# adalkiran/llama-nuts-and-bolts

Measured on AMD Instinct MI355X. Metric: decode tokens/s Llama-3.1-8B bf16 @1/2/4/8 MI355X; % HBM roofline, higher is better.
Workload: dtype bf16; 1 GPU; Llama-3.1-8B bf16, 1xMI355X, single-prompt greedy decode, seq_len=128 -> +125 tokens (configs[1]'s prompt, --steps 125); prompt_len=128, sequences_in_flight=1, parallelism=single GPU, mode=exact-order (token-id identical to the CPU reference path), reported_repeat=median, weight_bytes_resident=16060522496

## Files before the change

llama-nuts-and-bolts_amd/csrc/lnb_api.cpp:

```cpp
#include <hip/hip_runtime.h>
#include <algorithm>
#include <array>
#include <cmath>
#include <cstdarg>
#include <cstdio>
#include <cstdlib>
#include <cstring>
#include <chrono>
#include <dirent.h>
#include <unistd.h>
#include <deque>
#include <map>
#include <mutex>
#include <string>
#include <vector>
#include "../../include/lnb.h"
#include "lnb_device.h"
#include "lnb_knobs.h"
#include "lnb_kvcopy.h"
#include "lnb_rowpack.h"
#include "lnb_batchplan.h"
#include "lnb_rccl.h"
static_assert(LNB_MAX_SEQ_LEN == LNB_SEQ_MAX, "lnb.h and lnb_device.h disagree on the longest context");
static_assert(ROWPACK_MAX_W == LNB_BATCH_MAX, "lnb_rowpack.h and lnb_device.h disagree on the columns of a pass");
static_assert(BATCHPLAN_COLS == LNB_STREAM_COLS, "lnb_batchplan.h and lnb_device.h disagree on the sequences of a column group");
static_assert(LNB_MAX_FORK == KVC_MAX_DST, "lnb.h and lnb_kvcopy.h disagree on the destinations of a fork");
static_assert(LNB_MAX_TOP_K == LNB_TOKPROB_MAX_K, "lnb.h and lnb_device.h disagree on the largest top-k");
static_assert(LNB_MAX_DRAFT == LNB_SPEC_MAX_DRAFT && LNB_MAX_DRAFT + 1 <= LNB_STREAM_COLS, "a verify pass is one column group of at most 16 columns");

extern "C" {
hipError_t lnbk_gemv(const GemvParams* p, int rw, int nch, int epi, int norm, hipStream_t st);
hipError_t lnbk_attn(const AttnParams* p, hipStream_t st);
hipError_t lnbk_attn_rows(const AttnParams* p, int pos0, hipStream_t st);
int lnbk_attn_short_max_T(int hd);
size_t lnbk_attn_long_lds(int seq_len);
size_t lnbk_attn_long_layout_lds(int seq_len);
size_t lnbk_attn_one_lds(int seq_len, int hd);
hipError_t lnbk_exp_table(double* tab, float divisor, hipStream_t st);
hipError_t lnbk_gemm(const GemmParams* p, int epi, hipStream_t st);
hipError_t lnbk_rmsnorm_rows(const uint16_t* x, const uint16_t* w, uint16_t* out, int S, int K, float eps, hipStream_t st);
hipError_t lnbk_embed(const uint16_t* emb, const int32_t* tokens, uint16_t* x, int S, int dim, int vocab, int* err, hipStream_t st);
hipError_t lnbk_argmax(const uint16_t* logits, int V, int32_t* next_token, StepState* state, int32_t* out_tokens, int out_cap, int advance, hipStream_t st);
hipError_t lnbk_set_state(StepState* state, int pos, int n_out, int honour_stop, hipStream_t st);
hipError_t lnbk_set_stop(StepState* state, const int32_t* ids, int n, hipStream_t st);
hipError_t lnbk_advance_state(StepState* state, int rows, hipStream_t st);
hipError_t lnbk_tile(const uint16_t* src, uint16_t* dst, int rows, int K, int row_off, int chain, int RW, int NCH, int gather, hipStream_t st);
// ... 885 lines not shown

enum { K_QKV = 0, K_ATTN = 1, K_WO = 2, K_W13 = 3, K_W2 = 4, K_HEAD = 5, K_LAYER = 6 };
static bool use_mfma(int S) { return knob(Knob::PREFILL_MFMA) && S >= 16; }
static GemmParams gemm_of(const TiledDesc& t, const uint16_t* x, int K, int n_rows, int S, const StepState* st) {
    GemmParams g{}; g.w = t.w; g.rw = t.rw; g.nch = t.nch; g.x = x; g.K = K; g.n_rows = n_rows; g.S = S; g.st = st; g.w16 = t.w16; return g;
}
static hipError_t gemv_dispatch(const lnb_ctx* c, const GemvParams* g, int rw, int nch, int epi, int norm, hipStream_t st) {
    return c->mode == LNB_MODE_FAST ? lnbk_fast_gemv(g, rw, nch, epi, norm, st) : lnbk_gemv(g, rw, nch, epi, norm, st);
}
static hipError_t gemm_dispatch(int mode, const GemmParams* g, int epi, hipStream_t st) {
    if (mode == LNB_MODE_FAST && g->S >= knob(Knob::FAST_GEMM_MIN_ROWS)) { hipError_t e = lnbk_fast_gemm(g, epi, st); if (e != hipErrorNotSupported) return e; }
    if (knob(Knob::PREFILL_STREAM) && (g->K & 127) == 0 && (g->w16 || (knob(Knob::PREFILL_NATIVE) && g->w && (g->rw == 4 ? g->nch == 1 && (epi == EPI_STORE || epi == EPI_RESID) : g->rw >= 16))))
        return lnbk_gemm_stream(g, epi, g_num_cus, st);
    return lnbk_gemm(g, epi, st);
}
static int enqueue_layer_kernel(lnb_ctx* c, int l, int S, int which, hipStream_t st_other = nullptr, int lds_pad = 0) {
    lnb_model* m = c->m; const lnb_model_args& a = m->a; hipStream_t st = st_other ? st_other : c->stream;
    LayerW& L = m->layers[l - m->layer_begin];
    uint16_t* ck = c->ck[l - m->layer_begin]; uint16_t* cv = c->cv[l - m->layer_begin];
    uint16_t* const hbuf = m->whole(l) ? c->h : c->x;
    if (use_mfma(S) && which != K_ATTN) {
        switch (which) {
        case K_QKV: {
            HIPCHK(lnbk_rmsnorm_rows(c->x, L.attn_norm, c->xn, S, a.dim, a.norm_eps, st));
            GemmParams g = gemm_of(L.wqkv, c->xn, a.dim, L.wqkv.n_rows, S, c->st);
            g.cis = m->cis; g.q_out = c->q; g.cache_k = ck; g.cache_v = cv; g.seq_len = c->seq_len; g.q_dim = m->q_dim; g.kv_dim = m->kv_dim; g.head_dim = m->head_dim;
            HIPCHK(gemm_dispatch(c->mode, &g, EPI_QKV_ROPE, st)); return 0; }
        case K_WO: { GemmParams g = gemm_of(L.wo, c->att, m->q_dim, a.dim, S, c->st); g.out = hbuf; g.res = c->x; HIPCHK(gemm_dispatch(c->mode, &g, EPI_RESID, st)); return 0; }
        case K_W13: {
            HIPCHK(lnbk_rmsnorm_rows(hbuf, L.ffn_norm, c->xn, S, a.dim, a.norm_eps, st));
// ... 4 lines not shown
    }
    switch (which) {
    case K_QKV: {
        GemvParams g{}; g.w = L.wqkv.w; g.x = c->x; g.norm_w = L.attn_norm; g.norm_fb = c->zseq_count + 1; g.eps = a.norm_eps; g.K = a.dim; g.n_rows = L.wqkv.n_rows; g.S = S; g.st = c->st;
        g.cis = m->cis; g.q_out = c->q; g.cache_k = ck; g.cache_v = cv; g.seq_len = c->seq_len; g.q_dim = m->q_dim; g.kv_dim = m->kv_dim; g.head_dim = m->head_dim;
        g.sched = c->sched;
        set_grid(g, L.wqkv); HIPCHK(gemv_dispatch(c, &g, L.wqkv.rw, 1, EPI_QKV_ROPE, 1, st)); return 0; }
    case K_ATTN: {
        AttnParams ap{}; ap.q = c->q; ap.cache_k = ck; ap.cache_v = cv; ap.out = c->att; ap.st = c->st; ap.dbg = g_dbg;
        ap.S = S; ap.H = a.n_heads; ap.KVH = a.n_kv_heads; ap.hd = m->head_dim; ap.seq_len = c->seq_len;
        ap.lds_T = c->seq_len < c->attn_short_cap ? c->seq_len : c->attn_short_cap;
        ap.host_T = c->call_T;
        ap.divisor = bf_wide_h(bf_trunc_h((float)std::sqrt((double)m->head_dim)));
        ap.mfma = use_mfma(S) ? 1 : 0; ap.exp_tab = m->exp_tab;
        ap.causal = (c->attn_causal && S > 1) ? 1 : 0;
        ap.longctx = 0; ap.force_zseq = c->force_zseq & 1; ap.e_buf = c->e_buf; ap.z_part = c->z_part; ap.zseq_count = c->zseq_count; ap.cnt = c->attn_cnt;
        if (ap.mfma && c->sidx_jt > 0 && c->call_T > 0 && c->sidx_jt * 16 >= c->call_T) { ap.score_idx = c->score_idx; ap.sidx_jt = c->sidx_jt; }
        if (S == 1 && c->attn_long) {
            const bool one = (knob(Knob::ATTN_ONE) || (c->force_zseq & 12)) && !(c->force_zseq & 2) && c->sched == LNB_SCHED_LATENCY && m->head_dim % 16 == 0 &&
                             a.n_heads * (m->head_dim / 16) <= g_num_cus && lnbk_attn_one_lds(c->seq_len, m->head_dim) <= (size_t)160 * 1024;
            ap.longctx = one ? ((c->force_zseq & 4) ? 3 : 2) : 1;
        }
        if (c->attn_rows && ap.causal) {
            ap.e_buf = c->sp_e_buf; ap.z_part = c->sp_z_part; ap.force_zseq = c->rows_flags & 1;
            HIPCHK(lnbk_attn_rows(&ap, c->call_T - S, st)); return 0;
        }
        if (c->mode == LNB_MODE_FAST && ap.mfma) {
            hipError_t e = lnbk_fast_attn(&ap, st);
            if (e != hipErrorNotSupported) { HIPCHK(e); return 0; }
        }
        HIPCHK(lnbk_attn(&ap, st)); return 0; }
    case K_WO: {
        GemvParams o{}; o.w = L.wo.w; o.x = c->att; o.K = m->q_dim; o.n_rows = a.dim; o.S = S; o.st = c->st; o.out = hbuf; o.res = c->x; o.sched = c->sched;
        set_grid(o, L.wo); HIPCHK(gemv_dispatch(c, &o, L.wo.rw, 1, EPI_RESID, 0, st)); return 0; }
    case K_W13: {
        GemvParams f{}; f.w = L.w13.w; f.x = hbuf; f.norm_w = L.ffn_norm; f.norm_fb = c->zseq_count + 1; f.eps = a.norm_eps; f.K = a.dim; f.n_rows = m->ffn_hidden; f.S = S; f.st = c->st;
        f.out = c->ffn; f.silu = m->silu; f.sched = c->sched;
        set_grid(f, L.w13); HIPCHK(gemv_dispatch(c, &f, L.w13.rw, 2, EPI_SILU_MUL, 1, st)); return 0; }
    case K_W2: {
        GemvParams d{}; d.w = L.w2.w; d.x = c->ffn; d.K = m->ffn_hidden; d.n_rows = a.dim; d.S = S; d.st = c->st; d.out = c->x; d.res = hbuf; d.lds_pad = lds_pad; d.sched = c->sched; d.prio = knob(Knob::W2_PRIO);
        set_grid(d, L.w2); HIPCHK(gemv_dispatch(c, &d, L.w2.rw, 1, EPI_RESID, 0, st)); return 0; }
    }
    return fail("bad kernel id");
}
static int enqueue_layers(lnb_ctx* c, int S, bool with_cb) {
    lnb_model* m = c->m;
    for (int l = m->layer_begin; l < m->layer_end; l++) {
        auto t0 = std::chrono::steady_clock::now();
        for (int k = K_QKV; k <= K_W2; k++) {
            if (!(k <= K_WO ? m->has_attn(l) : k == K_W13 ? m->has_w13(l) : m->has_w2(l))) continue;
            if (enqueue_layer_kernel(c, l, S, k)) return -1;
        }
        if (with_cb && c->cb) {
            HIPCHK(hipStreamSynchronize(c->stream));
            double secs = std::chrono::duration<double>(std::chrono::steady_clock::now() - t0).count();
// ... 2129 lines not shown
```

llama-nuts-and-bolts_amd/csrc/lnb_device.h:

```cpp
#pragma once
#include <stdint.h>
#include <stddef.h>

#if defined(__HIPCC__)
#define LNB_HD __host__ __device__ __forceinline__
#else
#define LNB_HD inline
#endif

struct TiledDesc {
    uint16_t* w;
    int n_rows;
    int k;
    int rw;
    int nch;
    int n_blocks;
    uint16_t* w16;
};
LNB_HD size_t tiled_index(int n, int k, int c, int K, int RW, int NCH) {
    if (RW == 4) return ((((size_t)(n >> 2) * (size_t)(K >> 7) + (size_t)(k >> 7)) * 64 + (size_t)((n & 3) * 16 + (k & 15))) << 3) + (size_t)((k & 127) >> 4);
    size_t b = (size_t)(n / RW), r = (size_t)(n % RW), kc = (size_t)(k >> 3), e = (size_t)(k & 7);
    return ((((b * (size_t)(K >> 3) + kc) * (size_t)NCH + (size_t)c) * (size_t)RW + r) << 3) + e;
}
LNB_HD size_t tiled_elems(int n_rows, int K, int RW, int NCH) {
    if (RW == 4) return (size_t)((n_rows + 15) / 16) * 16 * (size_t)K;
    return (size_t)((n_rows + RW - 1) / RW) * (size_t)RW * (size_t)NCH * (size_t)K;
}

LNB_HD uint64_t lnb_splitmix64(uint64_t z) {
    z += 0x9E3779B97F4A7C15ULL;
    z = (z ^ (z >> 30)) * 0xBF58476D1CE4E5B9ULL;
    z = (z ^ (z >> 27)) * 0x94D049BB133111EBULL;
    return z ^ (z >> 31);
}
LNB_HD int32_t lnb_synth_isum(uint64_t base, uint64_t idx) {
    uint64_t a = lnb_splitmix64(base ^ idx);
    uint64_t b = lnb_splitmix64(a);
    int32_t s = 0;
    for (int i = 0; i < 4; i++) { s += (int32_t)((a >> (16 * i)) & 0xFFFF); s += (int32_t)((b >> (16 * i)) & 0xFFFF); }
    return s - 262140;
}

// ... 23 lines not shown
    uint16_t* out;
    const uint16_t* res;
    const float* silu;
    const float* cis;
    uint16_t* q_out;
    uint16_t* cache_k;
    uint16_t* cache_v;
    int seq_len;
    int q_dim, kv_dim, head_dim;
    long long* dbg;
    int dbg_full;
    int* norm_fb;
    int lds_pad;
    int prio;
    int sched;
};

struct GemmParams {
    const uint16_t* w;
    int rw, nch;
    const uint16_t* x;
    int K, n_rows, S;
    const StepState* st;
    uint16_t* out; const uint16_t* res; const float* silu;
    const float* cis; uint16_t* q_out; uint16_t* cache_k; uint16_t* cache_v; int seq_len, q_dim, kv_dim, head_dim;
    const uint16_t* w16;
    const struct BatchTab* btab; const struct BatchKV* bkv;
    uint16_t* out_xt;
    int rows_fastest;
};
// ... 12 lines not shown
    int mfma;
    const double* exp_tab;
    int longctx;
    int force_zseq;
    double* e_buf;
    double* z_part;
    int pw_floats;
    int* zseq_count;
    unsigned* cnt;
    const struct BatchTab* btab; const struct BatchKV* bkv; uint16_t* out_xt;
    uint64_t* score_idx;
    int sidx_jt;
    int touch;
    int causal;
    int head_major;
};
constexpr int LNB_ATTN_ROWS_MAX = 16;
struct AttnRowsParams {
    AttnParams a;
    int W;
    int row0;
    int pos0;
    int pos_off;
};

constexpr int LNB_BATCH_MAX = 128;
constexpr int LNB_SEQ_MAX = 131072;
constexpr int LNB_STREAM_COLS = 16;
LNB_HD size_t m16_index(int n, int k, int c, int K, int NCH) {
    const int t = n >> 4, i = n & 15, C = k >> 7, e = (k >> 4) & 7, m = (k >> 2) & 3, kk = k & 3;
// ... 110 lines not shown
```

llama-nuts-and-bolts_amd/csrc/lnb_kernels.hip:

```cpp
#include <hip/hip_runtime.h>
#include <cstdlib>
#include <type_traits>
#include "lnb_device.h"
#include "lnb_seqsum.h"

#define DEVINL __device__ __forceinline__

DEVINL float bf_lo(uint32_t u) { return __uint_as_float(u << 16); }
DEVINL float bf_hi(uint32_t u) { return __uint_as_float(u & 0xffff0000u); }
DEVINL float bf_wide(uint16_t b) { return __uint_as_float(((uint32_t)b) << 16); }
DEVINL uint16_t bf_trunc(float f) { return (uint16_t)(__float_as_uint(f) >> 16); }

DEVINL uint4 ld_nt_u4(const void* p) {
    typedef unsigned int u4v __attribute__((ext_vector_type(4)));
    u4v v = __builtin_nontemporal_load((const u4v*)p);
    return make_uint4(v.x, v.y, v.z, v.w);
}

DEVINL float mac8(float acc, const float4& xa, const float4& xb, const uint4& w) {
    acc = fmaf(xa.x, bf_lo(w.x), acc); acc = fmaf(xa.y, bf_hi(w.x), acc);
    acc = fmaf(xa.z, bf_lo(w.y), acc); acc = fmaf(xa.w, bf_hi(w.y), acc);
    acc = fmaf(xb.x, bf_lo(w.z), acc); acc = fmaf(xb.y, bf_hi(w.z), acc);
    acc = fmaf(xb.z, bf_lo(w.w), acc); acc = fmaf(xb.w, bf_hi(w.w), acc);
    return acc;
// ... 370 lines not shown
}

template <int NCH, int EPI, int PX = 1>
DEVINL void gemv_epilogue(const GemvParams& p, const float (&acc)[NCH], int m, int n, bool valid) {
    if (EPI == EPI_STORE) {
        if (valid) p.out[(size_t)m * p.n_rows + n] = bf_trunc(acc[0]);
    } else if (EPI == EPI_RESID) {
        if (valid) {
            size_t o = (size_t)m * p.n_rows + n;
            p.out[o] = bf_trunc(bf_wide(p.res[o]) + bf_wide(bf_trunc(acc[0])));
        }
    } else if (EPI == EPI_SILU_MUL) {
        if (valid) {
            uint16_t g = bf_trunc(acc[0]), u = bf_trunc(acc[NCH - 1]);
            uint16_t gs = bf_trunc(p.silu[g]);
            p.out[(size_t)m * p.n_rows + n] = bf_trunc(bf_wide(gs) * bf_wide(u));
        }
    } else if (EPI == EPI_QKV_ROPE) {
        const int pos = p.st->pos + m;
        const uint16_t mine = bf_trunc(acc[0]);
        const uint16_t other = (uint16_t)__shfl_xor((int)mine, PX);
        if (valid) {
            if (n < p.q_dim + p.kv_dim) {
                const int d = n % p.head_dim, i = d >> 1;
                const float2 cs = *(const float2*)(p.cis + ((size_t)pos * (p.head_dim >> 1) + i) * 2);
                const double cr = (double)cs.x, ci = (double)cs.y;
                uint16_t r16;
                if ((n & 1) == 0) { double a = (double)bf_wide(mine), bb = (double)bf_wide(other); r16 = bf_trunc((float)(a * cr - bb * ci)); }
                else              { double a = (double)bf_wide(other), bb = (double)bf_wide(mine); r16 = bf_trunc((float)(a * ci + bb * cr)); }
                if (n < p.q_dim) p.q_out[(size_t)m * p.q_dim + n] = r16;
                else {
// ... 635 lines not shown
                    acc = 0.0f; c = 0; blk += p.n_wg;
                }
            }
        }
    }
    asm volatile("s_waitcnt vmcnt(0) ; RING_RETIRE_ALL" ::: "memory");
    if (p.dbg && lane == 0) { long long* d_ = p.dbg + ((size_t)blockIdx.x * 8 + wave) * 4; d_[0] = clock64() - t_begin; d_[1] = 0; d_[2] = t_x; d_[3] = t_x; }
    LNB_WALL_EXIT();
}

constexpr int RL_SC = 4;
constexpr int RL_SLOTS = 3;
constexpr int RL_R = 12;
constexpr int RL_STAGE = 4 * RL_SC * 2048;
__host__ __device__ constexpr size_t rl_lds_bytes(int K) { return (size_t)RL_SLOTS * RL_STAGE + (size_t)K * 2; }
template <int EPI>
__global__ __launch_bounds__(512) void rowcast_lds_kernel(GemvParams p) {
    static_assert(RL_R == RL_SC * RL_SLOTS, "the helper's ring index and the product slot are static inside a three-stage unroll");
    extern __shared__ __attribute__((aligned(16))) char smem[];
    char* ring = smem;
    uint16_t* xb = (uint16_t*)(smem + RL_SLOTS * RL_STAGE);
    const long long t_begin = p.dbg ? clock64() : 0;
    const long long t_wall0 = p.dbg ? (long long)wall_clock64() : 0;
    long long t_x = 0, t_wait = 0, t_chain = 0;
    const int tid = threadIdx.x, lane = tid & 63;
    const int wave = __builtin_amdgcn_readfirstlane(tid >> 6), pair = wave & 3;
    const int K = p.K, S = p.S, nchunks = K >> 7, nst = nchunks / RL_SC;
    const int m = (S == 1) ? 0 : (int)(blockIdx.x % (unsigned)S);
    const int wg = (S == 1) ? (int)blockIdx.x : (int)(blockIdx.x / (unsigned)S);
    const int nb_mine = (p.n_blocks - wg + p.n_wg - 1) / p.n_wg;
    const int NS = nb_mine * nst;
    constexpr int RL_XU = 4;
    const uint16_t* xrow = p.x + (size_t)m * K;
    uint4 xv[RL_XU];
#pragma unroll
    for (int i = 0; i < RL_XU; i++) {
        const int u = tid + i * 512;
        xv[i] = *(const uint4*)(xrow + (size_t)(u < (K >> 3) ? u : 0) * 8);
    }
    __builtin_amdgcn_s_waitcnt(0x0F70);
    u32x4 buf[RL_R];
    const size_t tile_bytes = (size_t)nchunks * 1024;
    const char* sb = (const char*)p.w + ((size_t)wg * 4 + pair) * tile_bytes;
    const size_t blk_jump = (size_t)p.n_wg * 4 * tile_bytes - tile_bytes;
    const unsigned voff = (unsigned)lane * 16u;
    const int T = NS * RL_SC;
    int ic = 0, issued = 0;
    auto stage_x = [&]() {
#pragma unroll
        for (int i = 0; i < RL_XU; i++) {
            const int u = tid + i * 512;
            if (u < (K >> 3)) {
                const uint4 v = xv[i];
                const int k = u * 8, c = k >> 7, ii = (k & 127) >> 4, j0 = k & 15;
                uint16_t* d = xb + ((size_t)(c * 16 + j0) * 8 + ii);
                d[0] = (uint16_t)v.x; d[8] = (uint16_t)(v.x >> 16); d[16] = (uint16_t)v.y; d[24] = (uint16_t)(v.y >> 16);
                d[32] = (uint16_t)v.z; d[40] = (uint16_t)(v.z >> 16); d[48] = (uint16_t)v.w; d[56] = (uint16_t)(v.w >> 16);
            }
        }
        __syncthreads();
        if (p.dbg) t_x = clock64() - t_begin;
    };
#define RL_BARRIER() do { if (p.dbg_full) { const long long tb_ = clock64(); __builtin_amdgcn_s_barrier(); t_wait += clock64() - tb_; } else __builtin_amdgcn_s_barrier(); } while (0)
    auto products = [&](float4& pa, float4& pb, const u32x4& b, const uint4& xq) {
        pa = mul4(make_float4(bf_lo(xq.x), bf_hi(xq.x), bf_lo(xq.y), bf_hi(xq.y)), bf_lo(b.x), bf_hi(b.x), bf_lo(b.y), bf_hi(b.y));
        pb = mul4(make_float4(bf_lo(xq.z), bf_hi(xq.z), bf_lo(xq.w), bf_hi(xq.w)), bf_lo(b.z), bf_hi(b.z), bf_lo(b.w), bf_hi(b.w));
    };
    const char* xl = (const char*)xb + (size_t)(lane & 15) * 16;
    if (wave >= 4) {
        const int Th = T - RL_SC;
        auto advance = [&]() { sb += 1024; if (++ic == nchunks) { ic = 0; sb += blk_jump; } };
        auto issue_h = [&](u32x4& dst) {
            ld_nt_asm(dst, voff, sb);
            if (issued + 1 < Th) { issued++; advance(); if (issued == RL_SC) { for (int j = 0; j < RL_SC; j++) advance(); } }
        };
#pragma unroll
        for (int j = 0; j < RL_SC; j++) issue_h(buf[j]);
        stage_x();
#pragma unroll
        for (int j = RL_SC; j < RL_R; j++) issue_h(buf[j]);
        char* const dst0 = ring + (size_t)pair * (RL_SC * 2048) + (size_t)lane * 16;
        int c = 0;
        for (int it0 = 0; it0 <= NS; it0 += RL_SLOTS) {
#pragma unroll
            for (int u = 0; u < RL_SLOTS; u++) {
                const int it = it0 + u;
                if (it <= NS) {
                    if (it == 0 || it + 1 < NS) {
                        char* dst = dst0 + (size_t)(it == 0 ? 0 : (u + 1) % RL_SLOTS) * RL_STAGE;
#pragma unroll
                        for (int cc = 0; cc < RL_SC; cc++) {
                            u32x4& b = buf[u * RL_SC + cc];
                            asm volatile("s_waitcnt vmcnt(%1) ; RING_RETIRE %0" : "+v"(b) : "n"(RL_R - 1) : "memory");
                            const uint4 xq = *(const uint4*)(xl + (size_t)c * 256);
                            float4 pa, pb;
                            products(pa, pb, b, xq);
                            asm volatile("" : "+v"(pa.x), "+v"(pa.y), "+v"(pa.z), "+v"(pa.w), "+v"(pb.x), "+v"(pb.y), "+v"(pb.z), "+v"(pb.w));
                            issue_h(b);
                            *(float4*)(dst + cc * 2048) = pa; *(float4*)(dst + cc * 2048 + 1024) = pb;
                            if (++c == nchunks) c = 0;
                        }
                        if (it == 0) c = (2 * RL_SC) % nchunks;
                    }
                    __builtin_amdgcn_fence(__ATOMIC_RELEASE, "workgroup");
                    RL_BARRIER();
                }
            }
        }
        asm volatile("s_waitcnt vmcnt(0) ; RING_RETIRE_ALL" ::: "memory");
    } else {
        u32x4 cb[RL_SC];
#pragma unroll
        for (int j = 0; j < RL_SC; j++) ld_nt_asm(cb[j], voff, sb + (size_t)(RL_SC + j) * 1024);
        stage_x();
        const char* const src0 = ring + (size_t)pair * (RL_SC * 2048) + (size_t)lane * 16;
        {
            char* dst = ring + (size_t)pair * (RL_SC * 2048) + (size_t)lane * 16 + (size_t)1 * RL_STAGE;
#pragma unroll
            for (int cc = 0; cc < RL_SC; cc++) {
                if (cc == 0) asm volatile("s_waitcnt vmcnt(3) ; RING_RETIRE %0" : "+v"(cb[0]) :: "memory");
                if (cc == 1) asm volatile("s_waitcnt vmcnt(2) ; RING_RETIRE %0" : "+v"(cb[1]) :: "memory");
                if (cc == 2) asm volatile("s_waitcnt vmcnt(1) ; RING_RETIRE %0" : "+v"(cb[2]) :: "memory");
                if (cc == 3) asm volatile("s_waitcnt vmcnt(0) ; RING_RETIRE %0" : "+v"(cb[3]) :: "memory");
                const uint4 xq = *(const uint4*)(xl + (size_t)(RL_SC + cc) * 256);
                float4 pa, pb;
                products(pa, pb, cb[cc], xq);
                *(float4*)(dst + cc * 2048) = pa; *(float4*)(dst + cc * 2048 + 1024) = pb;
            }
            __builtin_amdgcn_fence(__ATOMIC_RELEASE, "workgroup");
            RL_BARRIER();
            __builtin_amdgcn_fence(__ATOMIC_ACQUIRE, "workgroup");
        }
        __builtin_amdgcn_s_setprio(3);
        if (p.dbg) { t_chain = clock64() - t_begin; t_wait = 0; }
        LNB_STAMP(6);
        float acc = 0.0f;
        float4 ba[2], bb[2];
        ba[0] = *(const float4*)src0; bb[0] = *(const float4*)(src0 + 1024);
        int sdone = 0, blk = wg;
// ... 1125 lines not shown
            }
        }
    } else {
        for (int c = 0; c <= nchunks; c += (VD + 1)) {
            __syncthreads(); __syncthreads(); __syncthreads(); __syncthreads();
            if constexpr (VD == 7) { __syncthreads(); __syncthreads(); __syncthreads(); __syncthreads(); }
        }
    }
    asm volatile("s_waitcnt vmcnt(0) ; RING_RETIRE_ALL" ::: "memory");
    ATT_STAMP(6);
    if (wave < 2) {
        const int r = wave * 64 + lane;
        if (r < HD) {
            const int d = attn_row_dim<HD>(r);
            if (bt && p.out_xt) p.out_xt[xt_group(i, p.H * HD) + xt_index(i & 15, h * HD + d)] = bf_trunc(acc);
            else p.out[((size_t)i * p.H + h) * HD + d] = bf_trunc(acc);
        }
    }
}

__host__ __device__ inline int gqa_tp(int lds_T) { return ((lds_T + 63) / 64) * 64 + 64; }
__host__ __device__ inline size_t gqa_lds_bytes(int lds_T, int hd, int G) { return (size_t)G * gqa_tp(lds_T) * 12 + (size_t)G * hd * 4 + 512 + 4 * 32 * (size_t)hd * 2; }
typedef float f32x2_t __attribute__((ext_vector_type(2)));
template <int HD> DEVINL void gqa_read_piece(uint32_t (&w)[8], float4 (&pq)[2], const char* vl, const float* pg, int q) {
    const char* vb = vl + ((q >> 2) & 3) * (32 * HD * 2) + (q & 3) * (8 * HD * 2);
    pq[0] = *(const float4*)(pg + q * 8); pq[1] = *(const float4*)(pg + q * 8 + 4);
#pragma unroll
    for (int u = 0; u < 8; u++) w[u] = *(const uint32_t*)(vb + u * (HD * 2));
}
DEVINL void gqa_add_piece(f32x2_t& a, const uint32_t (&w)[8], const float4 (&pq)[2]) {
#pragma unroll
// ... 185 lines not shown
}
struct AlSeq { int seq_len, T; const uint16_t* ck; const uint16_t* cv; size_t row; };
DEVINL AlSeq al_seq(const AttnParams& p, int h) {
    AlSeq a;
    const int s = blockIdx.z;
    a.seq_len = p.btab->seq_len[s]; a.ck = p.bkv->ck[s]; a.cv = p.bkv->cv[s]; a.row = (size_t)s * p.H + h;
    const int T = p.btab->st[s]->pos + 1;
    a.T = T < 1 ? 1 : (T > a.seq_len ? a.seq_len : T);
    return a;
}
template <bool BATCH> DEVINL int al_len(const AttnParams& p, const AlSeq& a) { if constexpr (BATCH) return a.seq_len; else return p.seq_len; }
template <bool BATCH> DEVINL int al_T(const AttnParams& p, const AlSeq& a) { if constexpr (BATCH) return a.T; else return p.st->pos + 1; }
template <bool BATCH> DEVINL const uint16_t* al_ck(const AttnParams& p, const AlSeq& a) { if constexpr (BATCH) return a.ck; else return p.cache_k; }
template <bool BATCH> DEVINL const uint16_t* al_cv(const AttnParams& p, const AlSeq& a) { if constexpr (BATCH) return a.cv; else return p.cache_v; }
template <bool BATCH> DEVINL size_t al_row(const AlSeq& a, int h) { if constexpr (BATCH) return a.row; else return (size_t)h; }
DEVINL void al_store(const AttnParams& p, int h, int hd_, int d, float acc) {
    const int s = blockIdx.z;
    if (p.out_xt) p.out_xt[xt_group(s, p.H * hd_) + xt_index(s & 15, h * hd_ + d)] = bf_trunc(acc);
    else p.out[((size_t)s * p.H + h) * hd_ + d] = bf_trunc(acc);
}
template <int HD, bool BATCH = false> __global__ __launch_bounds__(ALS_NT) void attn_long_scores_kernel(AttnParams p) {
    constexpr int NK = HD / 8;
    __shared__ __attribute__((aligned(16))) float qf[HD];
    __shared__ double wsum[ALS_NT / 64];
    const int tid = threadIdx.x;
    int h, blk; xcd_head_block(h, blk);
    [[maybe_unused]] AlSeq sq{}; if constexpr (BATCH) sq = al_seq(p, h);
    const int T = al_T<BATCH>(p, sq), j0 = blk * ALS_NT;
    if (j0 >= T) return;
    const int kvh = h / (p.H / p.KVH);
// ... 143 lines not shown
            if (it > 0) {
                const float* src = ring + (size_t)((it - 1) & 1) * ALP_SLOT + (size_t)d * ALP_BATCH + jj * 4;
                float4 a0 = *(const float4*)(src), a1 = *(const float4*)(src + 64);
#pragma unroll
                for (int c = 0; c < 4; c++) {
                    float pr[8] = {a0.x, a0.y, a0.z, a0.w, a1.x, a1.y, a1.z, a1.w};
                    if (c < 3) { a0 = *(const float4*)(src + (c + 1) * 128); a1 = *(const float4*)(src + (c + 1) * 128 + 64); }
                    asm volatile("" : "+v"(pr[0]), "+v"(pr[1]), "+v"(pr[2]), "+v"(pr[3]), "+v"(pr[4]), "+v"(pr[5]), "+v"(pr[6]), "+v"(pr[7]));
                    __builtin_amdgcn_sched_barrier(0);
                    chain128(acc, pr);
                }
            }
            __syncthreads();
        }
        ALP_STAMP(5);
        if (jj == 0) { if constexpr (BATCH) al_store(p, h, HD, ds * ALP_DS + d, acc); else p.out[(size_t)h * HD + ds * ALP_DS + d] = bf_trunc(acc); }
        ALP_STAMP(6);
    } else {
        auto produce = [&](const uint4 (&v)[4], int b) {
            float* dst = ring + (size_t)(b & 1) * ALP_SLOT + (size_t)(half8 * 8) * ALP_BATCH + ((prow >> 6) & 1) * 64 + (prow & 15) * 4 + ((prow >> 4) & 3);
#pragma unroll
            for (int r = 0; r < 4; r++) {
                const float pj = pw[b * ALP_BATCH + r * 128 + prow];
                const uint4 w = v[r];
                float* q = dst + r * 128;
                q[0 * ALP_BATCH] = pj * bf_lo(w.x); q[1 * ALP_BATCH] = pj * bf_hi(w.x); q[2 * ALP_BATCH] = pj * bf_lo(w.y); q[3 * ALP_BATCH] = pj * bf_hi(w.y);
                q[4 * ALP_BATCH] = pj * bf_lo(w.z); q[5 * ALP_BATCH] = pj * bf_hi(w.z); q[6 * ALP_BATCH] = pj * bf_lo(w.w); q[7 * ALP_BATCH] = pj * bf_hi(w.w);
            }
        };
        auto step = [&](int it, const uint4 (&cur)[4], uint4 (&nxt)[4]) {
            if (it <= nbatch) {
// ... 111 lines not shown
                double v[16];
#pragma unroll
                for (int u = 0; u < 16; u++) v[u] = E[j0 + u < T ? j0 + u : T - 1];
#pragma unroll
                for (int u = 0; u < 16; u++) z += (j0 + u < T) ? v[u] : 0.0;
            }
            if (lane == 0) { zsh[0] = z; if (p.zseq_count && ds == 0) atomicAdd(p.zseq_count, 1); }
        }
        if (wave >= 4) { load(v0, 0); load(v1, 1); load(v2, 2); }
        __syncthreads();
        run_pv(true, zsh[0]);
    }
    ALQ_STAMP(5);
    if (wave < 4 && (lane & 15) == 0) {
        if constexpr (BATCH) al_store(p, h, HD, ds * ALP_DS + 4 * wave + (lane >> 4), acc);
        else p.out[(size_t)h * HD + ds * ALP_DS + 4 * wave + (lane >> 4)] = bf_trunc(acc);
    }
    ALQ_STAMP(6);
#undef ALQ_STAMP
}

template <int HD, bool BATCH = false> __global__ __launch_bounds__(ALP_NT) void attn_long_pv2_kernel(AttnParams p) {
    if constexpr (BATCH) { if (p.btab->st[blockIdx.z]->pos + 1 <= 2 * ALP_BATCH) alp_eager_body<HD, true>(p); else alp_lazy_body<HD, true>(p); }
    else if (p.st->pos + 1 <= 2 * ALP_BATCH) alp_eager_body<HD>(p); else alp_lazy_body<HD>(p);
}

DEVINL int ar_pos(const AttnRowsParams& rp) { return (rp.pos0 >= 0 ? rp.pos0 : rp.a.btab ? rp.a.btab->st[0]->pos : rp.a.st->pos) + rp.pos_off; }
DEVINL int ar_T(const AttnRowsParams& rp, int pos, int i) { const int T = pos + i + 1; return T < 1 ? 1 : (T > rp.a.seq_len ? rp.a.seq_len : T); }
DEVINL const uint16_t* ar_ck(const AttnParams& p) { return p.btab ? p.bkv->ck[0] : p.cache_k; }
DEVINL const uint16_t* ar_cv(const AttnParams& p) { return p.btab ? p.bkv->cv[0] : p.cache_v; }
DEVINL void ar_store(const AttnRowsParams& rp, int row, int h, int hd_, int d, float acc) {
// ... 358 lines not shown
            if (it > 0) {
                const float* src = ring + (size_t)((it - 1) & 1) * ALP_SLOT + (size_t)d * ALP_BATCH + jj * 4;
                float4 a0 = *(const float4*)(src), a1 = *(const float4*)(src + 64);
#pragma unroll
                for (int c = 0; c < 4; c++) {
                    float pr[8] = {a0.x, a0.y, a0.z, a0.w, a1.x, a1.y, a1.z, a1.w};
                    if (c < 3) { a0 = *(const float4*)(src + (c + 1) * 128); a1 = *(const float4*)(src + (c + 1) * 128 + 64); }
                    asm volatile("" : "+v"(pr[0]), "+v"(pr[1]), "+v"(pr[2]), "+v"(pr[3]), "+v"(pr[4]), "+v"(pr[5]), "+v"(pr[6]), "+v"(pr[7]));
                    __builtin_amdgcn_sched_barrier(0);
                    chain128(acc, pr);
                }
            }
            __syncthreads();
        }
        AT1_STAMP(6);
        if (jj == 0) p.out[(size_t)h * HD + ds * ALP_DS + d] = bf_trunc(acc);
    } else {
        auto produce = [&](const uint4 (&v)[4], int b) {
            float* dst = ring + (size_t)(b & 1) * ALP_SLOT + (size_t)(half8 * 8) * ALP_BATCH + ((prow >> 6) & 1) * 64 + (prow & 15) * 4 + ((prow >> 4) & 3);
#pragma unroll
            for (int r = 0; r < 4; r++) {
                const float pj = pw[b * ALP_BATCH + r * 128 + prow];
                const uint4 w = v[r];
                float* q = dst + r * 128;
                q[0 * ALP_BATCH] = pj * bf_lo(w.x); q[1 * ALP_BATCH] = pj * bf_hi(w.x); q[2 * ALP_BATCH] = pj * bf_lo(w.y); q[3 * ALP_BATCH] = pj * bf_hi(w.y);
                q[4 * ALP_BATCH] = pj * bf_lo(w.z); q[5 * ALP_BATCH] = pj * bf_hi(w.z); q[6 * ALP_BATCH] = pj * bf_lo(w.w); q[7 * ALP_BATCH] = pj * bf_hi(w.w);
            }
        };
        auto step = [&](int it, const uint4 (&cur)[4], uint4 (&nxt)[4]) {
            if (it <= nbatch) {
                if (it < nbatch) { load(nxt, it + 3); produce(cur, it); }
// ... 497 lines not shown
    if constexpr (NCH == 1 && !NORM && (EPI == EPI_RESID || EPI == EPI_STORE)) {
        const int quad16 = p ? knob(Knob::W2_QUAD) : 0;
        if (rw == 16 && (!p || (quad16 && p->K % 128 == 0))) {
            const hipError_t e = either(quad16 == 2, launch_quad_t<16, 256, 4, 7, EPI, false>, launch_quad_t<16, 128, 4, 14, EPI, false>);
            if (p || e != hipSuccess) return e;
        }
    }
    if (rw == 16) return launch_chain_t<16, NCH, 8192, 2, 7, EPI, NORM>(p, st);
    if (rw == 32) return (NORM && NCH == 1) ? launch_chain_t<32, 1, 12288, 6, 5, EPI, NORM>(p, st) : launch_chain_t<32, NCH, 8192, 2, 7, EPI, NORM>(p, st);
    if (rw == 64) return launch_chain_t<64, NCH, 12288, 6, 8, EPI, NORM>(p, st);
    if constexpr (NCH == 2) if (rw == 56) return either(p && p->sched && knob(Knob::TP_W13), launch_chain_t<56, 2, 14336, 7, 6, EPI, NORM>, launch_chain_t<56, 2, 14336, 7, 8, EPI, NORM>);
    if constexpr (NCH == 2) if (rw == 28) return launch_chain_t<28, 2, 14336, 7, 8, EPI, NORM>(p, st);
    return hipErrorInvalidValue;
}

template <int EPI> static hipError_t launch_rowcast(const GemvParams* p, hipStream_t st) {
    auto kfn = rowcast_kernel<EPI>;
    auto kl = rowcast_lds_kernel<EPI>;
    if (!p) return raise_lds(kl, kfn);
    if ((p->K & 127) || p->K > 16384) return hipErrorInvalidValue;
    if (knob(Knob::ROWCAST_LDS) && !p->sched && p->K % (128 * RL_SC) == 0 && p->K >= 2 * 128 * RL_SC && rl_lds_bytes(p->K) + (size_t)(p->lds_pad > 0 ? p->lds_pad : 0) <= 160 * 1024) {
        hipLaunchKernelGGL(kl, dim3((unsigned)(p->S * p->n_wg)), dim3(512), rl_lds_bytes(p->K) + (size_t)(p->lds_pad > 0 ? p->lds_pad : 0), st, *p);
        return hipGetLastError();
    }
    hipLaunchKernelGGL(kfn, dim3((unsigned)(p->S * p->n_wg)), dim3(256), (size_t)p->K * 4 + (size_t)(p->lds_pad > 0 ? p->lds_pad : 0), st, *p);
    return hipGetLastError();
}

extern "C" hipError_t lnbk_gemv(const GemvParams* p, int rw, int nch, int epi, int norm, hipStream_t st) {
    if (rw == 4) {
        if (nch != 1 || norm) return hipErrorInvalidValue;
        if (epi == EPI_STORE) return launch_rowcast<EPI_STORE>(p, st);
        if (epi == EPI_RESID) return launch_rowcast<EPI_RESID>(p, st);
        return hipErrorInvalidValue;
    }
    if (nch == 2) {
        if (epi == EPI_SILU_MUL && norm) return launch_gemv_rw<EPI_SILU_MUL, true, 2>(p, rw, st);
        return hipErrorInvalidValue;
    }
// ... 433 lines not shown
```

llama-nuts-and-bolts_amd/csrc/lnb_knobs.h:

```cpp
#pragma once
#include <atomic>
#include <cstdlib>
#define LNB_KNOBS(X) \
     \
    X(RW_QKV, 0, LIVE, "rows per block of the resident wq|wk|wv layout (16 / 24 / 32 / 64; 0: by shape)") \
    X(RW_WO, 0, LIVE, "rows per block of the resident wo layout (4: row-broadcast; 0: by shape)") \
    X(RW_W13, 0, LIVE, "rows per block of the resident gate|up layout (28: the half-height band order, measurement; 0: by shape)") \
    X(RW_W2, 0, LIVE, "rows per block of the resident w2 layout (16 with W2_QUAD: measurement; 0: by shape)") \
    X(RW_OUT, 0, LIVE, "rows per block of the resident LM-head layout (0: by shape)") \
    X(RW_OP, 0, LIVE, "rows per block of a stand-alone lnb_op_linear operand (0: by shape)") \
     \
    X(PREFILL_MFMA, 1, ONCE, "0: calls of 16+ rows stay on the one-row kernels (what the parity tests compare the matrix-core forms with)") \
    X(PREFILL_STREAM, 1, ONCE, "0: prefill products on the LDS-tiled gemm_mfma_kernel, never the streaming feed") \
    X(PREFILL_NATIVE, 1, ONCE, "0: the streaming feed only from the matrix-core copy, not from the resident layouts") \
    X(GEMM_TILE, 0, ONCE, "force the gemm_mfma_kernel tile: 1 (16-row) / 64 / 128; 0: by tile count") \
    X(GS_NTW, 0, LIVE, "force gemm_stream_kernel's batch tiles per wave: 1 / 2 / 4") \
    X(GS_NTW_CHAIN, 0, ONCE, "the same, for the chain layouts only") \
    X(GS_TT, -1, LIVE, "two weight tiles per wave in gemm_stream_kernel: 0 never, 1 whenever the form exists, -1 by workgroup count") \
    X(GS_ORDER, -1, ONCE, "gemm_stream_kernel dispatch order: 1 row groups fastest, 0 tile groups fastest, -1 by row-group count") \
    X(GEMM_BLGP, 0, LIVE, "1 / 2: chain-layout prefill products through gemm_blgp_kernel (bit-exact, measured slower)") \
    X(NORM_ROWS_WIDE, 1, ONCE, "0: prefill RMSNorm on the one-wave rmsnorm_rows_kernel") \
    X(ATTN_MFMA2, 0, LIVE, "N > 0: prefill attention of N+ rows on the two-tile attn_mfma2_kernel (measured slower); 0: never") \
    X(ATTN_SIDX_MB, 4096, LIVE, "largest score-index scratch (MiB) the scores-kept prefill attention may allocate") \
    X(ATTN_SIDX_KEEP_MB, 256, LIVE, "a score-index scratch above this (MiB) is given back at the next one-token call") \
// ... 18 lines not shown
    X(FORK_SPLIT, 0, LIVE, "N > 1: kv_fork_kernel deals the destinations over N workgroup groups, each reading the source (measurement: slower from 1024 positions on)") \
     \
    X(FAST_GEMM_MIN_ROWS, 192, ONCE, "rows from which the tolerance mode uses its bf16 GEMM instead of the exact one") \
    X(FAST_GEMM_2WG, -1, ONCE, "bf16 GEMM batch tile: 1 = 128 rows and two workgroups per CU, 0 = 256 rows, -1 by row count") \
    X(FAST_RG, 0, ONCE, "force the rows per unit of the split-K GEMV: 8 / 16 / 32 / 64") \
    X(FAST_GRID_CAP, 2048, ONCE, "largest grid.x of the split-K GEMV") \
     \
    X(PIPELINE_GRAPH, 1, LIVE, "0: pipeline stages launch eagerly instead of replaying captured graphs") \
    X(PIPELINE_LOG_CAP, 1 << 16, LIVE, "entries of a pipeline stage's event log ring (the wrap-around test shrinks it)") \
     \
    X(NO_GRAPH, 0, LIVE, "1: greedy and batched decode launch every step eagerly") \
    X(GEMV_TIMING, 0, LIVE, "1: lnb_profile_kernel dumps the per-wave stamps of the profiled launch") \
    X(PROFILE_SAME_LAYER, 0, LIVE, "1: lnb_profile_kernel stays on one layer (weights served from the Infinity Cache)") \
    X(MEASURE_SKIP_TOKEN_KERNELS, 0, LIVE, "1: the decode step without its embedding and argmax launches (timing only: tokens are garbage)") \
    X(ROWCAST_LDS, 1, ONCE, "0: the row-broadcast GEMV always on the self-feeding rowcast_kernel") \
    X(TP_W13, 1, ONCE, "0: the throughput schedule keeps the eight-stage gate|up kernel (A/B)") \
    X(W2_QUAD, 0, LIVE, "1 / 2: a 16-row w2 layout on gemv_quad_kernel with 128- / 256-step stages (measurement only)") \
    X(W2_PRIO, 0, LIVE, "wave priority handed to the w2 launch of a block (measurement)") \
    X(W2_LDS_PAD, 28 * 1024, LIVE, "LDS padding of the w2 launch in the profiled w1|w3 + w2 pair (measurement)") \
    X(ATTN_GQA_DBG, 0, LIVE, "1: attn_gqa_kernel stamps the phases of one workgroup (lnbk_attn_gqa_dbg_dump prints them)")
enum KnobLife { ONCE, LIVE };
#define X(n, d, l, p) n,
enum class Knob { LNB_KNOBS(X) COUNT };
#undef X
#define X(n, d, l, p) {"LNB_" #n, d, l},
constexpr struct KnobInfo { const char* name; int dflt; KnobLife life; } LNB_KNOB_TABLE[] = {LNB_KNOBS(X)};
#undef X
inline int knob(Knob k) {
    const KnobInfo& i = LNB_KNOB_TABLE[(int)k];
    auto read = [&] { const char* s = getenv(i.name); return s && *s ? atoi(s) : i.dflt; };
// ... 7 lines not shown
```

llama-nuts-and-bolts_amd/lnb.py:

```python
import ctypes as C
import os
import subprocess

import numpy as np

_HERE = os.path.dirname(os.path.abspath(__file__))
_SO = os.environ.get("LNB_SO") or os.path.join(_HERE, "liblnb_hip.so")
_CSRC = os.path.join(_HERE, "csrc")


MODE_EXACT, MODE_FAST = 0, 1


class LnbError(RuntimeError):
    pass


def build(force=False):
    srcs = [os.path.join(_CSRC, f) for f in os.listdir(_CSRC) if f.endswith((".hip", ".cpp", ".h", ".hpp")) or f == "Makefile"]
    srcs.append(os.path.join(_HERE, "..", "include", "lnb.h"))
    if os.environ.get("LNB_SO"):
        return _SO
    if force or not os.path.exists(_SO) or any(os.path.getmtime(s) > os.path.getmtime(_SO) for s in srcs):
        subprocess.check_call(["make", "-C", _CSRC, "-s"])
# ... 918 lines not shown
    return out


_M64 = (1 << 64) - 1


def _splitmix64(z):
    z = (z + 0x9E3779B97F4A7C15) & _M64
    z = ((z ^ (z >> 30)) * 0xBF58476D1CE4E5B9) & _M64
    z = ((z ^ (z >> 27)) * 0x94D049BB133111EB) & _M64
    return z ^ (z >> 31)


def synth_tokens(seed, n, vocab):
    return np.array([_splitmix64(seed ^ ((i * 0x9E3779B97F4A7C15) & _M64)) % vocab for i in range(n)], dtype=np.int32)
```

Before: 239.1 tokens/s.

## Write attention and gate|up outputs in chain order so wo/w2 skip LDS x staging

For one-token exact-mode steps, attention and the w1|w3 SiLU epilogue now store their output vector in a permuted 'chain' order that matches the consumption order of the rowcast_lds GEMV. The wo and w2 launches then use a new kernel variant that loads x chunks straight from global memory alongside each weight chunk, instead of staging the whole x row into LDS first. This removes the x-staging prologue and K*2 bytes of LDS per workgroup, at the cost of extra global loads per chunk and more outstanding vmcnt. Producers and consumers have to agree on the permutation, which is gated by a live knob and a shared eligibility check.

```diff
diff --git a/llama-nuts-and-bolts_amd/csrc/lnb_api.cpp b/llama-nuts-and-bolts_amd/csrc/lnb_api.cpp
--- a/llama-nuts-and-bolts_amd/csrc/lnb_api.cpp
+++ b/llama-nuts-and-bolts_amd/csrc/lnb_api.cpp
@@ -30,6 +30,7 @@
 
 extern "C" {
 hipError_t lnbk_gemv(const GemvParams* p, int rw, int nch, int epi, int norm, hipStream_t st);
+int lnbk_rowcast_takes_lds(int K, int sched, int lds_pad);
 hipError_t lnbk_attn(const AttnParams* p, hipStream_t st);
 hipError_t lnbk_attn_rows(const AttnParams* p, int pos0, hipStream_t st);
 int lnbk_attn_short_max_T(int hd);
@@ -945,6 +946,14 @@
         return lnbk_gemm_stream(g, epi, g_num_cus, st);
     return lnbk_gemm(g, epi, st);
 }
+static bool x_chain_pair(const lnb_ctx* c, int l, int S, bool ffn) {
+    const lnb_model* m = c->m;
+    if (S != 1 || c->mode != LNB_MODE_EXACT || !knob(Knob::X_CHAIN_ORDER)) return false;
+    if (ffn ? !(m->has_w13(l) && m->has_w2(l)) : !m->has_attn(l)) return false;
+    const LayerW& L = m->layers[l - m->layer_begin];
+    const TiledDesc& t = ffn ? L.w2 : L.wo;
+    return t.rw == 4 && t.nch == 1 && lnbk_rowcast_takes_lds(ffn ? m->ffn_hidden : m->q_dim, c->sched, 0) != 0;
+}
 static int enqueue_layer_kernel(lnb_ctx* c, int l, int S, int which, hipStream_t st_other = nullptr, int lds_pad = 0) {
     lnb_model* m = c->m; const lnb_model_args& a = m->a; hipStream_t st = st_other ? st_other : c->stream;
     LayerW& L = m->layers[l - m->layer_begin];
@@ -979,6 +988,7 @@
         ap.divisor = bf_wide_h(bf_trunc_h((float)std::sqrt((double)m->head_dim)));
         ap.mfma = use_mfma(S) ? 1 : 0; ap.exp_tab = m->exp_tab;
         ap.causal = (c->attn_causal && S > 1) ? 1 : 0;
+        ap.out_chain = x_chain_pair(c, l, S, false) ? 1 : 0;
         ap.longctx = 0; ap.force_zseq = c->force_zseq & 1; ap.e_buf = c->e_buf; ap.z_part = c->z_part; ap.zseq_count = c->zseq_count; ap.cnt = c->attn_cnt;
         if (ap.mfma && c->sidx_jt > 0 && c->call_T > 0 && c->sidx_jt * 16 >= c->call_T) { ap.score_idx = c->score_idx; ap.sidx_jt = c->sidx_jt; }
         if (S == 1 && c->attn_long) {
@@ -997,13 +1007,15 @@
         HIPCHK(lnbk_attn(&ap, st)); return 0; }
     case K_WO: {
         GemvParams o{}; o.w = L.wo.w; o.x = c->att; o.K = m->q_dim; o.n_rows = a.dim; o.S = S; o.st = c->st; o.out = hbuf; o.res = c->x; o.sched = c->sched;
+        o.x_chain = x_chain_pair(c, l, S, false) ? 1 : 0;
         set_grid(o, L.wo); HIPCHK(gemv_dispatch(c, &o, L.wo.rw, 1, EPI_RESID, 0, st)); return 0; }
     case K_W13: {
         GemvParams f{}; f.w = L.w13.w; f.x = hbuf; f.norm_w = L.ffn_norm; f.norm_fb = c->zseq_count + 1; f.eps = a.norm_eps; f.K = a.dim; f.n_rows = m->ffn_hidden; f.S = S; f.st = c->st;
-        f.out = c->ffn; f.silu = m->silu; f.sched = c->sched;
+        f.out = c->ffn; f.silu = m->silu; f.sched = c->sched; f.out_chain = x_chain_pair(c, l, S, true) ? 1 : 0;
         set_grid(f, L.w13); HIPCHK(gemv_dispatch(c, &f, L.w13.rw, 2, EPI_SILU_MUL, 1, st)); return 0; }
     case K_W2: {
         GemvParams d{}; d.w = L.w2.w; d.x = c->ffn; d.K = m->ffn_hidden; d.n_rows = a.dim; d.S = S; d.st = c->st; d.out = c->x; d.res = hbuf; d.lds_pad = lds_pad; d.sched = c->sched; d.prio = knob(Knob::W2_PRIO);
+        d.x_chain = x_chain_pair(c, l, S, true) ? 1 : 0;
         set_grid(d, L.w2); HIPCHK(gemv_dispatch(c, &d, L.w2.rw, 1, EPI_RESID, 0, st)); return 0; }
     }
     return fail("bad kernel id");
diff --git a/llama-nuts-and-bolts_amd/csrc/lnb_device.h b/llama-nuts-and-bolts_amd/csrc/lnb_device.h
--- a/llama-nuts-and-bolts_amd/csrc/lnb_device.h
+++ b/llama-nuts-and-bolts_amd/csrc/lnb_device.h
@@ -26,6 +26,8 @@
     if (RW == 4) return (size_t)((n_rows + 15) / 16) * 16 * (size_t)K;
     return (size_t)((n_rows + RW - 1) / RW) * (size_t)RW * (size_t)NCH * (size_t)K;
 }
+
+LNB_HD int chain_index(int n) { return (n & ~127) | ((n & 15) << 3) | ((n >> 4) & 7); }
 
 LNB_HD uint64_t lnb_splitmix64(uint64_t z) {
     z += 0x9E3779B97F4A7C15ULL;
@@ -79,6 +81,8 @@
     int lds_pad;
     int prio;
     int sched;
+    int out_chain;
+    int x_chain;
 };
 
 struct GemmParams {
@@ -121,6 +125,7 @@
     int touch;
     int causal;
     int head_major;
+    int out_chain;
 };
 constexpr int LNB_ATTN_ROWS_MAX = 16;
 struct AttnRowsParams {
diff --git a/llama-nuts-and-bolts_amd/csrc/lnb_kernels.hip b/llama-nuts-and-bolts_amd/csrc/lnb_kernels.hip
--- a/llama-nuts-and-bolts_amd/csrc/lnb_kernels.hip
+++ b/llama-nuts-and-bolts_amd/csrc/lnb_kernels.hip
@@ -408,7 +408,7 @@
         if (valid) {
             uint16_t g = bf_trunc(acc[0]), u = bf_trunc(acc[NCH - 1]);
             uint16_t gs = bf_trunc(p.silu[g]);
-            p.out[(size_t)m * p.n_rows + n] = bf_trunc(bf_wide(gs) * bf_wide(u));
+            p.out[p.out_chain ? (size_t)chain_index(n) : (size_t)m * p.n_rows + n] = bf_trunc(bf_wide(gs) * bf_wide(u));
         }
     } else if (EPI == EPI_QKV_ROPE) {
         const int pos = p.st->pos + m;
@@ -1074,8 +1074,10 @@
 constexpr int RL_R = 12;
 constexpr int RL_STAGE = 4 * RL_SC * 2048;
 __host__ __device__ constexpr size_t rl_lds_bytes(int K) { return (size_t)RL_SLOTS * RL_STAGE + (size_t)K * 2; }
-template <int EPI>
+DEVINL void ld_x_asm(u32x4& dst, unsigned voff, const char* sbase) { asm volatile("global_load_dwordx4 %0, %1, %2 ; RING_LOAD" : "=&v"(dst) : "v"(voff), "s"(sbase) : "memory"); }
+template <int EPI, bool XCHAIN = false>
 __global__ __launch_bounds__(512) void rowcast_lds_kernel(GemvParams p) {
+    constexpr bool NOSTAGE = XCHAIN;
     static_assert(RL_R == RL_SC * RL_SLOTS, "the helper's ring index and the product slot are static inside a three-stage unroll");
     extern __shared__ __attribute__((aligned(16))) char smem[];
     char* ring = smem;
@@ -1093,12 +1095,14 @@
     constexpr int RL_XU = 4;
     const uint16_t* xrow = p.x + (size_t)m * K;
     uint4 xv[RL_XU];
-#pragma unroll
-    for (int i = 0; i < RL_XU; i++) {
-        const int u = tid + i * 512;
-        xv[i] = *(const uint4*)(xrow + (size_t)(u < (K >> 3) ? u : 0) * 8);
-    }
-    __builtin_amdgcn_s_waitcnt(0x0F70);
+    if constexpr (!NOSTAGE) {
+#pragma unroll
+        for (int i = 0; i < RL_XU; i++) {
+            const int u = tid + i * 512;
+            xv[i] = *(const uint4*)(xrow + (size_t)(u < (K >> 3) ? u : 0) * 8);
+        }
+        __builtin_amdgcn_s_waitcnt(0x0F70);
+    }
     u32x4 buf[RL_R];
     const size_t tile_bytes = (size_t)nchunks * 1024;
     const char* sb = (const char*)p.w + ((size_t)wg * 4 + pair) * tile_bytes;
@@ -1107,6 +1111,7 @@
     const int T = NS * RL_SC;
     int ic = 0, issued = 0;
     auto stage_x = [&]() {
+        if constexpr (NOSTAGE) { if (p.dbg) t_x = clock64() - t_begin; return; }
 #pragma unroll
         for (int i = 0; i < RL_XU; i++) {
             const int u = tid + i * 512;
@@ -1129,16 +1134,20 @@
     const char* xl = (const char*)xb + (size_t)(lane & 15) * 16;
     if (wave >= 4) {
         const int Th = T - RL_SC;
-        auto advance = [&]() { sb += 1024; if (++ic == nchunks) { ic = 0; sb += blk_jump; } };
-        auto issue_h = [&](u32x4& dst) {
+        const char* xs = (const char*)xrow;
+        const unsigned xoff = (unsigned)(lane & 15) * 16u;
+        u32x4 xr[NOSTAGE ? RL_R : 1];
+        auto advance = [&]() { sb += 1024; xs += 256; if (++ic == nchunks) { ic = 0; sb += blk_jump; xs = (const char*)xrow; } };
+        auto issue_h = [&](u32x4& dst, u32x4& xdst) {
             ld_nt_asm(dst, voff, sb);
+            if constexpr (NOSTAGE) ld_x_asm(xdst, xoff, xs);
             if (issued + 1 < Th) { issued++; advance(); if (issued == RL_SC) { for (int j = 0; j < RL_SC; j++) advance(); } }
         };
 #pragma unroll
-        for (int j = 0; j < RL_SC; j++) issue_h(buf[j]);
+        for (int j = 0; j < RL_SC; j++) issue_h(buf[j], xr[NOSTAGE ? j : 0]);
         stage_x();
 #pragma unroll
-        for (int j = RL_SC; j < RL_R; j++) issue_h(buf[j]);
+        for (int j = RL_SC; j < RL_R; j++) issue_h(buf[j], xr[NOSTAGE ? j : 0]);
         char* const dst0 = ring + (size_t)pair * (RL_SC * 2048) + (size_t)lane * 16;
         int c = 0;
         for (int it0 = 0; it0 <= NS; it0 += RL_SLOTS) {
@@ -1151,12 +1160,19 @@
 #pragma unroll
                         for (int cc = 0; cc < RL_SC; cc++) {
                             u32x4& b = buf[u * RL_SC + cc];
-                            asm volatile("s_waitcnt vmcnt(%1) ; RING_RETIRE %0" : "+v"(b) : "n"(RL_R - 1) : "memory");
-                            const uint4 xq = *(const uint4*)(xl + (size_t)c * 256);
+                            u32x4& bx = xr[NOSTAGE ? u * RL_SC + cc : 0];
+                            uint4 xq;
+                            if constexpr (NOSTAGE) {
+                                asm volatile("s_waitcnt vmcnt(%2) ; RING_RETIRE %0 %1" : "+v"(b), "+v"(bx) : "n"(2 * RL_R - 2) : "memory");
+                                xq = make_uint4(bx.x, bx.y, bx.z, bx.w);
+                            } else {
+                                asm volatile("s_waitcnt vmcnt(%1) ; RING_RETIRE %0" : "+v"(b) : "n"(RL_R - 1) : "memory");
+                                xq = *(const uint4*)(xl + (size_t)c * 256);
+                            }
                             float4 pa, pb;
                             products(pa, pb, b, xq);
                             asm volatile("" : "+v"(pa.x), "+v"(pa.y), "+v"(pa.z), "+v"(pa.w), "+v"(pb.x), "+v"(pb.y), "+v"(pb.z), "+v"(pb.w));
-                            issue_h(b);
+                            issue_h(b, bx);
                             *(float4*)(dst + cc * 2048) = pa; *(float4*)(dst + cc * 2048 + 1024) = pb;
                             if (++c == nchunks) c = 0;
                         }
@@ -1169,20 +1185,33 @@
         }
         asm volatile("s_waitcnt vmcnt(0) ; RING_RETIRE_ALL" ::: "memory");
     } else {
-        u32x4 cb[RL_SC];
-#pragma unroll
-        for (int j = 0; j < RL_SC; j++) ld_nt_asm(cb[j], voff, sb + (size_t)(RL_SC + j) * 1024);
+        u32x4 cb[RL_SC], cx[NOSTAGE ? RL_SC : 1];
+#pragma unroll
+        for (int j = 0; j < RL_SC; j++) {
+            ld_nt_asm(cb[j], voff, sb + (size_t)(RL_SC + j) * 1024);
+            if constexpr (NOSTAGE) ld_x_asm(cx[j], (unsigned)(lane & 15) * 16u, (const char*)xrow + (size_t)(RL_SC + j) * 256);
+        }
         stage_x();
         const char* const src0 = ring + (size_t)pair * (RL_SC * 2048) + (size_t)lane * 16;
         {
             char* dst = ring + (size_t)pair * (RL_SC * 2048) + (size_t)lane * 16 + (size_t)1 * RL_STAGE;
 #pragma unroll
             for (int cc = 0; cc < RL_SC; cc++) {
-                if (cc == 0) asm volatile("s_waitcnt vmcnt(3) ; RING_RETIRE %0" : "+v"(cb[0]) :: "memory");
-                if (cc == 1) asm volatile("s_waitcnt vmcnt(2) ; RING_RETIRE %0" : "+v"(cb[1]) :: "memory");
-                if (cc == 2) asm volatile("s_waitcnt vmcnt(1) ; RING_RETIRE %0" : "+v"(cb[2]) :: "memory");
-                if (cc == 3) asm volatile("s_waitcnt vmcnt(0) ; RING_RETIRE %0" : "+v"(cb[3]) :: "memory");
-                const uint4 xq = *(const uint4*)(xl + (size_t)(RL_SC + cc) * 256);
+                uint4 xq;
+                if constexpr (NOSTAGE) {
+                    u32x4& bx = cx[NOSTAGE ? cc : 0];
+                    if (cc == 0) asm volatile("s_waitcnt vmcnt(6) ; RING_RETIRE %0 %1" : "+v"(cb[0]), "+v"(bx) :: "memory");
+                    if (cc == 1) asm volatile("s_waitcnt vmcnt(4) ; RING_RETIRE %0 %1" : "+v"(cb[1]), "+v"(bx) :: "memory");
+                    if (cc == 2) asm volatile("s_waitcnt vmcnt(2) ; RING_RETIRE %0 %1" : "+v"(cb[2]), "+v"(bx) :: "memory");
+                    if (cc == 3) asm volatile("s_waitcnt vmcnt(0) ; RING_RETIRE %0 %1" : "+v"(cb[3]), "+v"(bx) :: "memory");
+                    xq = make_uint4(bx.x, bx.y, bx.z, bx.w);
+                } else {
+                    if (cc == 0) asm volatile("s_waitcnt vmcnt(3) ; RING_RETIRE %0" : "+v"(cb[0]) :: "memory");
+                    if (cc == 1) asm volatile("s_waitcnt vmcnt(2) ; RING_RETIRE %0" : "+v"(cb[1]) :: "memory");
+                    if (cc == 2) asm volatile("s_waitcnt vmcnt(1) ; RING_RETIRE %0" : "+v"(cb[2]) :: "memory");
+                    if (cc == 3) asm volatile("s_waitcnt vmcnt(0) ; RING_RETIRE %0" : "+v"(cb[3]) :: "memory");
+                    xq = *(const uint4*)(xl + (size_t)(RL_SC + cc) * 256);
+                }
                 float4 pa, pb;
                 products(pa, pb, cb[cc], xq);
                 *(float4*)(dst + cc * 2048) = pa; *(float4*)(dst + cc * 2048 + 1024) = pb;
@@ -2338,7 +2367,7 @@
         if (r < HD) {
             const int d = attn_row_dim<HD>(r);
             if (bt && p.out_xt) p.out_xt[xt_group(i, p.H * HD) + xt_index(i & 15, h * HD + d)] = bf_trunc(acc);
-            else p.out[((size_t)i * p.H + h) * HD + d] = bf_trunc(acc);
+            else p.out[p.out_chain ? (size_t)chain_index(h * HD + d) : ((size_t)i * p.H + h) * HD + d] = bf_trunc(acc);
         }
     }
 }
@@ -2554,6 +2583,7 @@
 template <bool BATCH> DEVINL const uint16_t* al_ck(const AttnParams& p, const AlSeq& a) { if constexpr (BATCH) return a.ck; else return p.cache_k; }
 template <bool BATCH> DEVINL const uint16_t* al_cv(const AttnParams& p, const AlSeq& a) { if constexpr (BATCH) return a.cv; else return p.cache_v; }
 template <bool BATCH> DEVINL size_t al_row(const AlSeq& a, int h) { if constexpr (BATCH) return a.row; else return (size_t)h; }
+DEVINL size_t alp_out_index(const AttnParams& p, int n) { return (size_t)(p.out_chain ? chain_index(n) : n); }
 DEVINL void al_store(const AttnParams& p, int h, int hd_, int d, float acc) {
     const int s = blockIdx.z;
     if (p.out_xt) p.out_xt[xt_group(s, p.H * hd_) + xt_index(s & 15, h * hd_ + d)] = bf_trunc(acc);
@@ -2727,7 +2757,7 @@
             __syncthreads();
         }
         ALP_STAMP(5);
-        if (jj == 0) { if constexpr (BATCH) al_store(p, h, HD, ds * ALP_DS + d, acc); else p.out[(size_t)h * HD + ds * ALP_DS + d] = bf_trunc(acc); }
+        if (jj == 0) { if constexpr (BATCH) al_store(p, h, HD, ds * ALP_DS + d, acc); else p.out[alp_out_index(p, h * HD + ds * ALP_DS + d)] = bf_trunc(acc); }
         ALP_STAMP(6);
     } else {
         auto produce = [&](const uint4 (&v)[4], int b) {
@@ -2869,7 +2899,7 @@
     ALQ_STAMP(5);
     if (wave < 4 && (lane & 15) == 0) {
         if constexpr (BATCH) al_store(p, h, HD, ds * ALP_DS + 4 * wave + (lane >> 4), acc);
-        else p.out[(size_t)h * HD + ds * ALP_DS + 4 * wave + (lane >> 4)] = bf_trunc(acc);
+        else p.out[alp_out_index(p, h * HD + ds * ALP_DS + 4 * wave + (lane >> 4))] = bf_trunc(acc);
     }
     ALQ_STAMP(6);
 #undef ALQ_STAMP
@@ -3258,7 +3288,7 @@
             __syncthreads();
         }
         AT1_STAMP(6);
-        if (jj == 0) p.out[(size_t)h * HD + ds * ALP_DS + d] = bf_trunc(acc);
+        if (jj == 0) p.out[alp_out_index(p, h * HD + ds * ALP_DS + d)] = bf_trunc(acc);
     } else {
         auto produce = [&](const uint4 (&v)[4], int b) {
             float* dst = ring + (size_t)(b & 1) * ALP_SLOT + (size_t)(half8 * 8) * ALP_BATCH + ((prow >> 6) & 1) * 64 + (prow & 15) * 4 + ((prow >> 4) & 3);
@@ -3786,15 +3816,24 @@
     return hipErrorInvalidValue;
 }
 
+extern "C" int lnbk_rowcast_takes_lds(int K, int sched, int lds_pad) {
+    return knob(Knob::ROWCAST_LDS) && !sched && (K & 127) == 0 && K <= 16384 && K % (128 * RL_SC) == 0 && K >= 2 * 128 * RL_SC && rl_lds_bytes(K) + (size_t)(lds_pad > 0 ? lds_pad : 0) <= 160 * 1024;
+}
 template <int EPI> static hipError_t launch_rowcast(const GemvParams* p, hipStream_t st) {
     auto kfn = rowcast_kernel<EPI>;
     auto kl = rowcast_lds_kernel<EPI>;
-    if (!p) return raise_lds(kl, kfn);
+    auto kx = rowcast_lds_kernel<EPI, true>;
+    if (!p) return raise_lds(kl, kx, kfn);
     if ((p->K & 127) || p->K > 16384) return hipErrorInvalidValue;
-    if (knob(Knob::ROWCAST_LDS) && !p->sched && p->K % (128 * RL_SC) == 0 && p->K >= 2 * 128 * RL_SC && rl_lds_bytes(p->K) + (size_t)(p->lds_pad > 0 ? p->lds_pad : 0) <= 160 * 1024) {
-        hipLaunchKernelGGL(kl, dim3((unsigned)(p->S * p->n_wg)), dim3(512), rl_lds_bytes(p->K) + (size_t)(p->lds_pad > 0 ? p->lds_pad : 0), st, *p);
+    if (lnbk_rowcast_takes_lds(p->K, p->sched, p->lds_pad)) {
+        const size_t pad = (size_t)(p->lds_pad > 0 ? p->lds_pad : 0);
+        if (p->x_chain) {
+            if (p->S != 1) return hipErrorInvalidValue;
+            hipLaunchKernelGGL(kx, dim3((unsigned)p->n_wg), dim3(512), (size_t)RL_SLOTS * RL_STAGE + pad, st, *p);
+        } else hipLaunchKernelGGL(kl, dim3((unsigned)(p->S * p->n_wg)), dim3(512), rl_lds_bytes(p->K) + pad, st, *p);
         return hipGetLastError();
     }
+    if (p->x_chain) return hipErrorInvalidValue;
     hipLaunchKernelGGL(kfn, dim3((unsigned)(p->S * p->n_wg)), dim3(256), (size_t)p->K * 4 + (size_t)(p->lds_pad > 0 ? p->lds_pad : 0), st, *p);
     return hipGetLastError();
 }
diff --git a/llama-nuts-and-bolts_amd/csrc/lnb_knobs.h b/llama-nuts-and-bolts_amd/csrc/lnb_knobs.h
--- a/llama-nuts-and-bolts_amd/csrc/lnb_knobs.h
+++ b/llama-nuts-and-bolts_amd/csrc/lnb_knobs.h
@@ -56,6 +56,7 @@
     X(PROFILE_SAME_LAYER, 0, LIVE, "1: lnb_profile_kernel stays on one layer (weights served from the Infinity Cache)") \
     X(MEASURE_SKIP_TOKEN_KERNELS, 0, LIVE, "1: the decode step without its embedding and argmax launches (timing only: tokens are garbage)") \
     X(ROWCAST_LDS, 1, ONCE, "0: the row-broadcast GEMV always on the self-feeding rowcast_kernel") \
+    X(X_CHAIN_ORDER, 1, LIVE, "0: the attention and gate|up rows of a one-token step stay in natural order and wo / w2 transpose them in the LDS (A/B, parity test)") \
     X(TP_W13, 1, ONCE, "0: the throughput schedule keeps the eight-stage gate|up kernel (A/B)") \
     X(W2_QUAD, 0, LIVE, "1 / 2: a 16-row w2 layout on gemv_quad_kernel with 128- / 256-step stages (measurement only)") \
     X(W2_PRIO, 0, LIVE, "wave priority handed to the w2 launch of a block (measurement)") \
diff --git a/llama-nuts-and-bolts_amd/lnb.py b/llama-nuts-and-bolts_amd/lnb.py
--- a/llama-nuts-and-bolts_amd/lnb.py
+++ b/llama-nuts-and-bolts_amd/lnb.py
@@ -956,3 +956,7 @@
 
 def synth_tokens(seed, n, vocab):
     return np.array([_splitmix64(seed ^ ((i * 0x9E3779B97F4A7C15) & _M64)) % vocab for i in range(n)], dtype=np.int32)
+
+
+def chain_index(n):
+    return (n & ~127) | ((n & 15) << 3) | ((n >> 4) & 7)
```

Result: no change. 241.2 tokens/s, median of 6 (+0.9%).
